# DJjjjhao/FIRA-ICSE

Hardware: NVIDIA H100
Metric: train_commits_per_sec (higher is better)
Workload: dtype bf16

## Files before the change

### fira_icse_b200/csrc/head.cu

```cuda
#include "common.cuh"
#include "fira_b200.h"

namespace {

constexpr int D = 256;
constexpr int TMAX = 32;

__device__ __forceinline__ long src_row(const int* __restrict__ ranges, int b, int S, int s) {
  if (!ranges) return (long)b * S + s;
  const int* r = ranges + 4 * b;
  if (s < r[1]) return r[0] + s;
  s -= r[1];
  return s < r[3] ? (long)(r[2] + s) : -1;
}

template <typename T>
__global__ void __launch_bounds__(256) copy_scores_fwd_kernel(const T* __restrict__ src, const T* __restrict__ tgt,
                                                              const float* __restrict__ w_res,
                                                              const float* __restrict__ b_res_p,
                                                              const unsigned char* __restrict__ src_mask,
                                                              const unsigned char* __restrict__ row_mask,
                                                              const int* __restrict__ ranges,
                                                              float* __restrict__ sc, int B, int Tn, int S) {
  pdl_wait(); pdl_trigger();
// ... 130 lines not shown
struct MaxSum { float m, s; };
__device__ __forceinline__ MaxSum ms_merge(MaxSum a, MaxSum b) {
  const float m = fmaxf(a.m, b.m);
  MaxSum r;
  r.m = m;
  r.s = (a.s == 0.f ? 0.f : a.s * expf(a.m - m)) + (b.s == 0.f ? 0.f : b.s * expf(b.m - m));
  return r;
}
__device__ __forceinline__ MaxSum ms_warp(MaxSum v) {
#pragma unroll
  for (int o = 16; o > 0; o >>= 1) {
    MaxSum u;
    u.m = __shfl_xor_sync(0xffffffffu, v.m, o);
    u.s = __shfl_xor_sync(0xffffffffu, v.s, o);
    v = ms_merge(v, u);
  }
  return v;
}
struct ArgMax { float v; int i; };
__device__ __forceinline__ ArgMax am_better(ArgMax a, ArgMax b) {
  return (b.v > a.v || (b.v == a.v && b.i < a.i)) ? b : a;
}

template <typename T>
__global__ void __launch_bounds__(256) head_fwd_kernel(const T* __restrict__ logits, long ldl,
                                                       const float* __restrict__ sc, const float* __restrict__ gate_logit,
                                                       const unsigned char* __restrict__ mem_mask,
                                                       const int* __restrict__ label, float* __restrict__ stats,
                                                       float* __restrict__ nll, int* __restrict__ argmax_out, int Tn,
                                                       int V, int S) {
  pdl_wait(); pdl_trigger();
  __shared__ MaxSum sh_ms[8];
  __shared__ ArgMax sh_am[8];
  __shared__ float bc[8];
  const long row = blockIdx.x;
  const int b = (int)(row / Tn);
  const int lane = threadIdx.x & 31, warp = threadIdx.x >> 5;
  const T* lrow = logits + row * ldl;
  const float* srow = sc + row * S;
  const unsigned char* mrow = mem_mask + (long)b * S;

  const int lab_row = label[row];
  const bool need_vocab = argmax_out != nullptr || (lab_row != 0 && lab_row < V);
  MaxSum v{-INFINITY, 0.f};
  if (need_vocab) {
    const int V8 = V >> 3;
    for (int g = threadIdx.x; g < V8; g += blockDim.x) {
      float x[8];
      Act<T>::load8(lrow + (long)g * 8, x);
      float m8 = x[0];
#pragma unroll
      for (int i = 1; i < 8; ++i) m8 = fmaxf(m8, x[i]);
      if (m8 > v.m) { v.s *= expf(v.m - m8); v.m = m8; }
#pragma unroll
      for (int i = 0; i < 8; ++i) v.s += expf(x[i] - v.m);
    }
    for (int j = V8 * 8 + threadIdx.x; j < V; j += blockDim.x) { MaxSum u{Act<T>::ld(lrow + j), 1.f}; v = ms_merge(v, u); }
  } else if (threadIdx.x == 0) v = MaxSum{0.f, 1.f};
  v = ms_warp(v);
  if (lane == 0) sh_ms[warp] = v;
  __syncthreads();
  if (warp == 0) { MaxSum u = lane < 8 ? sh_ms[lane] : MaxSum{-INFINITY, 0.f}; u = ms_warp(u); if (lane == 0) { bc[0] = u.m; bc[1] = u.s; } }
  __syncthreads();
  MaxSum c{-INFINITY, 0.f};
  for (int j = threadIdx.x; j < S; j += blockDim.x) { MaxSum u{mrow[j] ? srow[j] : kMaskFill, 1.f}; c = ms_merge(c, u); }
  c = ms_warp(c);
  if (lane == 0) sh_ms[warp] = c;
  __syncthreads();
  if (warp == 0) { MaxSum u = lane < 8 ? sh_ms[lane] : MaxSum{-INFINITY, 0.f}; u = ms_warp(u); if (lane == 0) { bc[2] = u.m; bc[3] = u.s; } }
  __syncthreads();
  const float vmax = bc[0], vsum = bc[1], cmax = bc[2], csum = bc[3];
  const float gl0 = gate_logit[row * 2], gl1 = gate_logit[row * 2 + 1];
  const float gm = fmaxf(gl0, gl1);
  const float e0 = expf(gl0 - gm), e1 = expf(gl1 - gm);
  const float g0 = e0 / (e0 + e1), g1 = e1 / (e0 + e1);

  if (threadIdx.x == 0) {
    const int lab = label[row];
    float p = 1.f;
    if (lab != 0) {
      if (lab < V) p = g0 * (expf(Act<T>::ld(lrow + lab) - vmax) / vsum);
      else {
        const int s = lab - V;
        p = s < S ? g1 * (expf((mrow[s] ? srow[s] : kMaskFill) - cmax) / csum) : 0.f;
      }
    }
    float* st = stats + row * 8;
    st[0] = vmax; st[1] = vsum; st[2] = cmax; st[3] = csum; st[4] = g0; st[5] = g1; st[6] = p; st[7] = 0.f;
    nll[row] = lab != 0 ? -logf(fminf(fmaxf(p, 1e-10f), 1.f)) : 0.f;
  }
  if (argmax_out) {
    ArgMax best{-INFINITY, 0x7fffffff};
    const float iv = 1.f / vsum, ic = 1.f / csum;
    for (int j = threadIdx.x; j < V + S; j += blockDim.x) {
      float p;
      if (j < V) p = g0 * (expf(Act<T>::ld(lrow + j) - vmax) * iv);
      else { const int s = j - V; p = g1 * (expf((mrow[s] ? srow[s] : kMaskFill) - cmax) * ic); }
      ArgMax cand{logf(fminf(fmaxf(p, 1e-10f), 1.f)), j};
      best = am_better(best, cand);
    }
#pragma unroll
    for (int o = 16; o > 0; o >>= 1) {
      ArgMax u{__shfl_xor_sync(0xffffffffu, best.v, o), __shfl_xor_sync(0xffffffffu, best.i, o)};
      best = am_better(best, u);
    }
    if (lane == 0) sh_am[warp] = best;
    __syncthreads();
    if (threadIdx.x == 0) {
      ArgMax r = sh_am[0];
      for (int q = 1; q < 8; ++q) r = am_better(r, sh_am[q]);
      argmax_out[row] = r.i;
    }
  }
}

template <typename T>
__global__ void __launch_bounds__(256) head_bwd_kernel(const T* __restrict__ logits, long ldl,
                                                       const float* __restrict__ sc,
                                                       const unsigned char* __restrict__ mem_mask,
                                                       const int* __restrict__ label, const float* __restrict__ stats,
                                                       const float* __restrict__ upstream, T* __restrict__ d_logits,
                                                       float* __restrict__ d_sc, float* __restrict__ d_gate_logit,
                                                       unsigned char* __restrict__ row_active, int Tn, int V, int S) {
  pdl_wait(); pdl_trigger();
  const long row = blockIdx.x;
  const int b = (int)(row / Tn);
  const float* st = stats + row * 8;
  const float vmax = st[0], vsum = st[1], cmax = st[2], csum = st[3], g0 = st[4], g1 = st[5], p = st[6];
  const int lab = label[row];
  const float up = *upstream;
  const bool live = lab != 0 && p >= 1e-10f && p <= 1.f;
  const bool vocab = live && lab < V;
  const bool copy = live && lab >= V;
  T* drow = d_logits + row * ldl;
  const T* lrow = logits + row * ldl;
  const int V8 = V >> 3;
  if (vocab) {
    const float iv = 1.f / vsum;
    for (int g = threadIdx.x; g < V8; g += blockDim.x) {
      float x[8];
      Act<T>::load8(lrow + (long)g * 8, x);
#pragma unroll
      for (int i = 0; i < 8; ++i) x[i] = up * (expf(x[i] - vmax) * iv - (g * 8 + i == lab ? 1.f : 0.f));
      Act<T>::store8(drow + (long)g * 8, x);
    }
    for (int j = V8 * 8 + threadIdx.x; j < V; j += blockDim.x) {
      float pv = expf(Act<T>::ld(lrow + j) - vmax) * iv;
      Act<T>::st(drow + j, up * (pv - (j == lab ? 1.f : 0.f)));
    }
  } else {
    const float z[8] = {0.f, 0.f, 0.f, 0.f, 0.f, 0.f, 0.f, 0.f};
    for (int g = threadIdx.x; g < V8; g += blockDim.x) Act<T>::store8(drow + (long)g * 8, z);
    for (int j = V8 * 8 + threadIdx.x; j < V; j += blockDim.x) Act<T>::st(drow + j, 0.f);
  }
  const float* srow = sc + row * S;
  const unsigned char* mrow = mem_mask + (long)b * S;
  float* dsrow = d_sc + row * S;
  if (copy) {
    const float ic = 1.f / csum;
    for (int j = threadIdx.x; j < S; j += blockDim.x) {
      float pc = expf((mrow[j] ? srow[j] : kMaskFill) - cmax) * ic;
      dsrow[j] = mrow[j] ? up * (pc - (j == lab - V ? 1.f : 0.f)) : 0.f;
    }
  } else {
    for (int j = threadIdx.x; j < S; j += blockDim.x) dsrow[j] = 0.f;
  }
  if (threadIdx.x == 0) {
    float d0 = 0.f, d1 = 0.f;
    if (vocab) { d0 = up * (g0 - 1.f); d1 = up * g1; }
    if (copy) { d0 = up * g0; d1 = up * (g1 - 1.f); }
    d_gate_logit[row * 2] = d0; d_gate_logit[row * 2 + 1] = d1;
    row_active[row] = copy ? 1 : 0;
  }
}
// ... 632 lines not shown
int fira_copy_scores_bwd(const void* src_proj, const void* tgt_proj, const float* w_res, const float* d_scores,
                         const unsigned char* row_active, void* d_src_proj, float* d_tgt_proj, float* d_w_res,
                         float* d_b_res, int B, int T_len, int S, int dim, int dtype, void* stream) {
  return copy_scores_bwd_impl(src_proj, tgt_proj, w_res, d_scores, row_active, nullptr, d_src_proj, d_tgt_proj, d_w_res,
                              d_b_res, B, T_len, S, dim, dtype, stream);
}

int fira_copy_scores_packed_fwd(const void* src_proj, const void* tgt_proj, const float* w_res, const float* b_res,
                                const int* ranges, const unsigned char* src_mask, const unsigned char* row_mask,
                                float* scores, int B, int T_len, int S, int dim, int dtype, void* stream) {
  FIRA_CHECK_ARG(ranges, FIRA_ERR_ARG, "copy_scores_packed_fwd: null ranges");
  return copy_scores_fwd_impl(src_proj, tgt_proj, w_res, b_res, src_mask, row_mask, ranges, scores, B, T_len, S, dim,
                              dtype, stream);
}

int fira_copy_scores_packed_bwd(const void* src_proj, const void* tgt_proj, const float* w_res, const float* d_scores,
                                const unsigned char* row_active, const int* ranges, void* d_src_proj, float* d_tgt_proj,
                                float* d_w_res, float* d_b_res, int B, int T_len, int S, int dim, int dtype, void* stream) {
  FIRA_CHECK_ARG(ranges, FIRA_ERR_ARG, "copy_scores_packed_bwd: null ranges");
  return copy_scores_bwd_impl(src_proj, tgt_proj, w_res, d_scores, row_active, ranges, d_src_proj, d_tgt_proj, d_w_res,
                              d_b_res, B, T_len, S, dim, dtype, stream);
}

int fira_pointer_mix_nll_fwd(const void* logits, long ld_logits, const float* copy_scores, const float* gate_logits,
                             const unsigned char* mem_mask, const int* label, float* stats, float* nll,
                             int* argmax_out, long rows, int T_len, int V, int S, int dtype, void* stream) {
  FIRA_CHECK_ARG(rows >= 0 && T_len > 0 && V > 0 && S > 0, FIRA_ERR_SHAPE, "pointer_mix_nll_fwd: shape");
  FIRA_CHECK_ARG(fira_aligned16(logits) && ld_logits % 8 == 0, FIRA_ERR_ALIGN,
                 "pointer_mix_nll_fwd: logits must be 16-byte aligned with a leading dimension that is a multiple of 8");
  if (rows == 0) return FIRA_OK;
  DISPATCH_T(dtype, launch_k(head_fwd_kernel<T>, dim3((unsigned)rows), dim3(256), 0, (cudaStream_t)stream, 
      (const T*)logits, ld_logits, copy_scores, gate_logits, mem_mask, label, stats, nll, argmax_out, T_len, V, S);)
  FIRA_CHECK_LAUNCH("fira_pointer_mix_nll_fwd");
  return FIRA_OK;
}

int fira_pointer_mix_nll_bwd(const void* logits, long ld_logits, const float* copy_scores,
                             const unsigned char* mem_mask, const int* label, const float* stats,
                             const float* upstream, void* d_logits, float* d_copy_scores, float* d_gate_logits,
                             unsigned char* row_active, long rows, int T_len, int V, int S, int dtype, void* stream) {
  FIRA_CHECK_ARG(rows >= 0 && T_len > 0 && V > 0 && S > 0, FIRA_ERR_SHAPE, "pointer_mix_nll_bwd: shape");
  FIRA_CHECK_ARG(fira_aligned16(logits) && fira_aligned16(d_logits) && ld_logits % 8 == 0, FIRA_ERR_ALIGN,
                 "pointer_mix_nll_bwd: logits / d_logits must be 16-byte aligned with a leading dimension that is a multiple of 8");
  if (rows == 0) return FIRA_OK;
  DISPATCH_T(dtype, launch_k(head_bwd_kernel<T>, dim3((unsigned)rows), dim3(256), 0, (cudaStream_t)stream, 
      (const T*)logits, ld_logits, copy_scores, mem_mask, label, stats, upstream, (T*)d_logits, d_copy_scores,
      d_gate_logits, row_active, T_len, V, S);)
  FIRA_CHECK_LAUNCH("fira_pointer_mix_nll_bwd");
  return FIRA_OK;
}

static int sample_impl(const void* logits, long ld_logits, const float* copy_scores, const float* gate_logits,
                       const unsigned char* mem_mask, const int* copy_src, const uint64_t* seed, const int* first_index,
                       const float* uniforms, float temperature, int top_k, float top_p, int eos_id, int pad_id,
                       int* next_tok, int* seq, int* raw, float* token_logprob, unsigned char* tok_mask, long ld_out,
                       int pos, unsigned char* finished, int* length, float* logprob, int B, int N, int V, int S,
                       const int* prefix, int ld_prefix, const int* prefix_len, int no_repeat, int min_len, int dtype,
                       void* stream) {
  FIRA_CHECK_ARG(!prefix || (prefix_len && ld_prefix > pos), FIRA_ERR_ARG,
                 "pointer_mix_sample_prefix: null prefix_len or ld_prefix %d <= pos %d", ld_prefix, pos);
  FIRA_CHECK_ARG(no_repeat >= 0 && min_len >= 0, FIRA_ERR_ARG,
                 "pointer_mix_sample_rules: no_repeat_ngram %d / min_length %d < 0", no_repeat, min_len);
  FIRA_CHECK_ARG((!no_repeat && !min_len) || ld_out <= TMAX, FIRA_ERR_SHAPE,
                 "pointer_mix_sample_rules: ld_out %ld > %d", ld_out, TMAX);
  FIRA_CHECK_ARG(B >= 0 && N > 0 && V > 0 && S > 0 && V + S <= 0x7FFF, FIRA_ERR_SHAPE,
                 "pointer_mix_sample: shape (B %d, N %d, V %d, S %d; V + S must be <= 32767)", B, N, V, S);
  FIRA_CHECK_ARG(pos >= 0 && ld_out >= pos + 2, FIRA_ERR_SHAPE, "pointer_mix_sample: pos %d, ld_out %ld", pos, ld_out);
  FIRA_CHECK_ARG(temperature > 0.f && temperature <= 3.4e38f, FIRA_ERR_ARG, "pointer_mix_sample: temperature %g",
                 (double)temperature);
  FIRA_CHECK_ARG(top_k >= 0, FIRA_ERR_ARG, "pointer_mix_sample: top_k %d < 0", top_k);
  FIRA_CHECK_ARG(top_p > 0.f && top_p <= 1.f, FIRA_ERR_ARG, "pointer_mix_sample: top_p %g not in (0, 1]", (double)top_p);
  FIRA_CHECK_ARG(uniforms || (seed && first_index), FIRA_ERR_ARG, "pointer_mix_sample: seed / first_index missing");
// ... 215 lines not shown
```

### fira_icse_b200/data.py

```python
import json
import os
import random

import numpy as np
import torch
from torch.utils.data import Dataset

from ._lib import host_call

num_train, num_valid, num_test = 75000, 8000, 7661
lemmatization = {"added": "add", "fixed": "fix", "removed": "remove",
                 "adding": "add", "fixing": "fix", "removing": "remove"}
RAW_FILES = ["difftoken", "diffatt", "diffmark", "msg", "variable", "change", "ast",
             "edge_change_code", "edge_change_ast", "edge_ast_code", "edge_ast"]


def _lower(tok, upper):
    return tok if tok in upper else tok.lower()


def _to_ids(tokens, vocab, upper):
    out = []
    for t in tokens:
        t = _lower(t, upper)
# ... 301 lines not shown

    def __len__(self):
        n = len(self.indices)
        return n // self.B if self.drop_last else -(-n // self.B)

    def _choose_dims(self, need):
        need = tuple(int(x) for x in need)
        if need in self.shapes or self.max_shapes is None or len(self.shapes) < self.max_shapes:
            self.shapes[need] = self.shapes.get(need, 0) + 1
            return need
        fits = [s for s in self.shapes if all(a >= b for a, b in zip(s, need))]
        if self.packed and not fits:
            self.shapes[need] = 1
            return need
        best = min(fits, key=sum) if fits else self.lens
        self.shapes[best] = self.shapes.get(best, 0) + 1
        return best

    def gather(self, index, slot=None):
        slot = self.slots[0] if slot is None else slot
        index = np.ascontiguousarray(index, dtype=np.int64)
        if self.packed:
            from . import packed as P
            need = self.tables.dims(index)
            want = tuple(P._round_up(need[i], self.row_buckets[i]) for i in range(4))
            return P.gather_packed(self.tables, index, self.V, slot, pad_dims=self._choose_dims(want))
        b = len(index)
        n0, n1, n2 = self.lens
        t = self.tab
        dims = np.zeros(3, np.int32)
        host_call("fira_host_batch_dims", t["sou"].ctypes.data, t["sub_token"].ctypes.data,
                  t["ast_change"].ctypes.data, index.ctypes.data, b, n0, n1, n2, *self.multiples, dims.ctypes.data)
        dims = np.asarray(self._choose_dims(dims), np.int32)
        nnz = np.zeros(1, np.int32)
        host_call("fira_host_gather_batch", t["sou"].ctypes.data, t["tar"].ctypes.data, t["mark"].ctypes.data,
                  t["ast_change"].ctypes.data, t["tar_label"].ctypes.data, t["sub_token"].ctypes.data,
                  self.deg.ctypes.data, self.col.ctypes.data, self.val.ctypes.data, self.edge_ptr.ctypes.data,
                  index.ctypes.data, b, n0, n1, n2, self.msg_len, self.V, dims.ctypes.data,
                  slot.sou.data_ptr(), slot.tar.data_ptr(), slot.mark.data_ptr(), slot.ast_change.data_ptr(),
                  slot.tar_label.data_ptr(), slot.sub_token.data_ptr(), slot.rowptr.data_ptr(), slot.col.data_ptr(),
                  slot.val.data_ptr(), self.edge_cap, nnz.ctypes.data)
        c0, c1, c2 = (int(x) for x in dims)
        e = int(nnz[0])
        slot.batch = [slot.sou[:b * c0].view(b, c0), slot.tar[:b * self.msg_len].view(b, self.msg_len), None,
                      slot.mark[:b * c0].view(b, c0), slot.ast_change[:b * c2].view(b, c2),
                      (slot.rowptr[:b * (c0 + c1 + c2) + 1], slot.col[:e], slot.val[:e]),
                      slot.tar_label[:b * self.msg_len].view(b, self.msg_len), slot.sub_token[:b * c1].view(b, c1)]
        return slot.batch
# ... 71 lines not shown
```

### fira_icse_b200/engine.py

```python
import os

import torch
import torch.distributed as dist

from . import optim as _optim
from .graph import PackedEdges
from .optim import FlatAdam
from .packed import PackedBatch
from .parallel import FlatGradBucket

ID_KEYS = ("sou", "tar", "mark", "ast_change", "tar_label", "sub_token")


class _Captured:

    def __init__(self, shapes, B, n_nodes, cap, dev):
        self.ids = {k: torch.zeros((B, n), dtype=torch.int64, device=dev) for k, n in zip(ID_KEYS, shapes)}
        self.rowptr = torch.zeros(B * n_nodes + 1, dtype=torch.int32, device=dev)
        self.col = torch.zeros(cap, dtype=torch.int32, device=dev)
        self.val = torch.zeros(cap, dtype=torch.float32, device=dev)
        self.B, self.n_nodes, self.cap = B, n_nodes, cap
        self.graph = None
        self.grads = None


class _CapturedPacked:

    def __init__(self, pb, cap, dev):
        def z(t, n=None):
            return torch.zeros(t.shape if n is None else (n,), dtype=t.dtype, device=dev)
        t = {k: z(getattr(pb, k)) for k in PackedBatch.FIELDS if k not in ("col", "val")}
        t["col"], t["val"] = z(pb.col, cap), z(pb.val, cap)
        self.pb = PackedBatch(pb.B, pb.Rc, pb.Rs, pb.Ra, pb.S, pb.T, cap, pb.chunks, **t)
        self.B, self.cap = pb.B, cap
        self.graph = None
        self.grads = None
        self.packed = True

    def copy_from(self, pb):
        for k in PackedBatch.FIELDS:
            src, dst = getattr(pb, k), getattr(self.pb, k)
            if k in ("col", "val"):
                dst[:src.numel()].copy_(src, non_blocking=True)
            else:
                dst.copy_(src, non_blocking=True)


class _OptimizerPair:

    def __init__(self, pair):
        self.pair = pair

    def step(self):
        for o in self.pair:
            o.step()

# ... 326 lines not shown
```

### fira_icse_b200/ops.py

```python
import ctypes
import os

import torch

from . import _lib
from . import optim as _optim
from ._lib import FIRA_BF16, FIRA_F32, call

D = 256

if hasattr(torch.autograd.graph, "set_warn_on_accumulate_grad_stream_mismatch"):
    torch.autograd.graph.set_warn_on_accumulate_grad_stream_mismatch(False)


def _stream():
    return torch.cuda.current_stream().cuda_stream


def _ptr(t, off=0):
    if t is None:
        return None
    return t.data_ptr() + off * t.element_size()


# ... 689 lines not shown

class HeadFn(torch.autograd.Function):

    @staticmethod
    def forward(ctx, want_argmax, bf16, pf, memory, dec, mem_mask, label, Wout, bout, Ws, Wt, Wres, bres, Wp, bp,
                pk=None):
        _require_cuda(memory, dec, Wout)
        B, T = dec.shape[0], dec.shape[1]
        S = pk.S if pk is not None else memory.shape[1]
        V = Wout.shape[0]
        Mt, Ms = B * T, memory.shape[0] * memory.shape[1]
        pr = Prec(bf16)
        if pf is not None and pf.event is not None:
            torch.cuda.current_stream().wait_event(pf.event)
            pf.fork.join()
            pr.wcache.update(pf.wcache)
        dev = dec.device
        f32 = dict(dtype=torch.float32, device=dev)
        st = _stream()
        memory2 = memory.contiguous().to(pr.tdt).view(Ms, D)
        dec2 = dec.contiguous().to(pr.tdt).view(Mt, D)
        dec32 = dec2 if not pr.bf16 else dec2.float()
        ldl = _ld_logits(V)
        logits = pr.empty((Mt, ldl), dev)
        pr.linear(dec2, Wout, bout, out=logits, ld_out=ldl)
        row_mask = None if want_argmax else (label >= V).to(torch.uint8)
        src, tgt, sc = copy_scores_fwd(pr, memory2, dec2, Ws, Wt, Wres, bres, B, T, S, src_mask=mem_mask,
                                       row_mask=row_mask, ranges=pk.ranges if pk is not None else None)
        gl = linear(dec32, Wp, bp)
        stats = torch.empty((Mt, 8), **f32)
        nll = torch.empty((Mt,), **f32)
        amax = torch.empty((Mt,), dtype=torch.int32, device=dev) if want_argmax else None
        call("fira_pointer_mix_nll_fwd", _ptr(logits), ldl, _ptr(sc), _ptr(gl), _ptr(mem_mask), _ptr(label),
             _ptr(stats), _ptr(nll), _ptr(amax), Mt, T, V, S, pr.code, st)
        ctx.misc = (pr, memory2, dec2, dec32, mem_mask, label, logits, ldl, src, tgt, sc, stats, B, T, S, V,
                    memory.dtype, dec.dtype, pk, memory.shape)
        ctx.save_for_backward(Wout, Ws, Wt, Wres, Wp, bout, bres, bp)
        loss_sum = colsum(nll, 1, Mt, 1).view(())
        ids = amax.view(B, T) if want_argmax else None
        nll2 = nll.view(B, T)
        ctx.mark_non_differentiable(*([nll2, ids] if ids is not None else [nll2]))
        return loss_sum, nll2, ids

    @staticmethod
    def backward(ctx, g_loss, g_nll, g_ids):
        (pr, memory2, dec2, dec32, mem_mask, label, logits, ldl, src, tgt, sc, stats, B, T, S, V,
         mem_dt, dec_dt, pk, mem_shape) = ctx.misc
        Wout, Ws, Wt, Wres, Wp, bout, bres, bp = ctx.saved_tensors
        Mt, Ms = B * T, memory2.shape[0]
        dev = dec2.device
        f32 = dict(dtype=torch.float32, device=dev)
        st = _stream()
        up = g_loss.contiguous().float()
        dlogits = pr.empty((Mt, ldl), dev)
        dsc = torch.empty((B, T, S), **f32)
        dgl = torch.empty((Mt, 2), **f32)
        active = torch.empty((Mt,), dtype=torch.uint8, device=dev)
        call("fira_pointer_mix_nll_bwd", _ptr(logits), ldl, _ptr(sc), _ptr(mem_mask), _ptr(label), _ptr(stats),
             _ptr(up), _ptr(dlogits), _ptr(dsc), _ptr(dgl), _ptr(active), Mt, T, V, S, pr.code, st)
        d_src = pr.empty((Ms, D), dev)
        d_tgt = torch.zeros((Mt, D), **f32)
        d_wres = _gdest(Wres, (1, D), zero=True)
        d_bres = _gdest(bres, (1,), zero=True)
        if pk is not None:
            call("fira_zero_pad_rows", _ptr(d_src), D, D, _ptr(pk.off), B, pk.Rc, pk.Rs, pr.code, st)
            call("fira_copy_scores_packed_bwd", _ptr(src), _ptr(tgt), _ptr(Wres), _ptr(dsc), _ptr(active), _ptr(pk.ranges),
                 _ptr(d_src), _ptr(d_tgt), _ptr(d_wres), _ptr(d_bres), B, T, S, D, pr.code, st)
        else:
            call("fira_copy_scores_bwd", _ptr(src), _ptr(tgt), _ptr(Wres), _ptr(dsc), _ptr(active), _ptr(d_src),
                 _ptr(d_tgt), _ptr(d_wres), _ptr(d_bres), B, T, S, D, pr.code, st)
        fork = Fork(dev)
        with fork(d_src, memory2):
            d_Ws = pr.linear_dw(d_src, D, memory2, D, Ms, D, D, out=_gdest(Ws, (D, D)))
        with fork(dlogits, dec2):
            d_bout = _gdest(bout, (V,), zero=True)
            d_Wout = pr.linear_dw(dlogits, ldl, dec2, D, Mt, V, D, out=_gdest(Wout, (V, D)), dbias=d_bout)
        with fork(dgl, dec32, d_tgt):
            d_bp = colsum(dgl, 2, Mt, 2, out=_gdest(bp, (2,), zero=True))
            d_Wp = linear_dw(dgl, 2, dec32, D, Mt, 2, D, out=_gdest(Wp, (2, D)))
            d_Wt = linear_dw(d_tgt, D, dec32, D, Mt, D, D, out=_gdest(Wt, (D, D)))
        d_mem = pr.linear_dx(d_src, D, Ws, Ms)
        if pr.bf16:
            d_dec = torch.empty((Mt, D), **f32)
            gemm_tc(dlogits, ldl, 1, pr.w(Wout), D, 0, d_dec, D, Mt, D, V,
                    splits=_tc_splits(_ceil(Mt, 128), _ceil(V, 64)))
        else:
            d_dec = linear_dx(dlogits, ldl, Wout, Mt)
        linear_dx(dgl, 2, Wp, Mt, out=d_dec, accumulate=True)
        linear_dx(d_tgt, D, Wt, Mt, out=d_dec, accumulate=True)
        fork.join()
        return (None, None, None, d_mem.view(mem_shape).to(mem_dt), d_dec.view(B, T, D).to(dec_dt), None, None, d_Wout,
                d_bout, d_Ws, d_Wt, d_wres, d_bres, d_Wp, d_bp, None)


class LinearFn(torch.autograd.Function):

    @staticmethod
    def forward(ctx, x, W, b):
        _require_cuda(x, W)
        N, K = W.shape
        x2 = x.contiguous().float().view(-1, K)
        M = x2.shape[0]
        ld = (N + 3) // 4 * 4
        out = torch.empty((M, ld), dtype=torch.float32, device=x.device)
        linear(x2, W, b, out=out, ld_out=ld)
        ctx.save_for_backward(x2, W)
        ctx.has_bias = b is not None
        ctx.shape = x.shape
        return out[:, :N].view(*x.shape[:-1], N)

# ... 46 lines not shown
```

### fira_icse_b200/packed.py

```python
import numpy as np
import torch

from ._lib import host_call

SEGMENT_BUCKETS = (1024, 512, 512, 64)


class PackedBatch:

    FIELDS = ("code", "mark", "pos", "sub", "ast", "off", "ranges", "mem_mask", "tar", "label", "tar_mask",
              "rowptr", "col", "val")

    def __init__(self, B, Rc, Rs, Ra, S, T, nnz, chunks=4, **tensors):
        self.B, self.Rc, self.Rs, self.Ra, self.S, self.T, self.nnz = B, Rc, Rs, Ra, S, T, nnz
        self.chunks = int(chunks)
        for k in self.FIELDS:
            setattr(self, k, tensors[k])

    @property
    def shape_key(self):
        return (self.B, self.Rc, self.Rs, self.Ra, self.S, self.chunks)

    @property
    def rows(self):
        return self.Rc + self.Rs + self.Ra

    @property
    def mem_rows(self):
        return self.Rc + self.Rs

    def to(self, device, non_blocking=True):
        t = {k: getattr(self, k).to(device, non_blocking=non_blocking) for k in self.FIELDS}
        return PackedBatch(self.B, self.Rc, self.Rs, self.Ra, self.S, self.T, self.nnz, self.chunks, **t)

    def h2d_bytes(self):
        return sum(getattr(self, k).numel() * getattr(self, k).element_size() for k in self.FIELDS)


def _round_up(x, m):
    return max(m, -(-int(x) // m) * m)


class PackedTables:

    ID_KEYS = ("sou", "tar", "mark", "ast_change", "tar_label", "sub_token")

    def __init__(self, dataset):
        d = dataset.d
        self.tab = {k: np.ascontiguousarray(d[k], dtype=np.int32) for k in self.ID_KEYS}
        self.deg = np.ascontiguousarray(d["deg"], dtype=np.uint8)
        self.col = np.ascontiguousarray(d["col"], dtype=np.int16)
        self.val = np.ascontiguousarray(d["val"], dtype=np.float64)
        self.edge_ptr = np.ascontiguousarray(d["edge_ptr"], dtype=np.int64)
        self.lens = (dataset.diff_len, dataset.sub_token_len, dataset.ast_change_len)
        self.msg_len = dataset.msg_len
        self.n = len(self.tab["sou"])

    def dims(self, index):
        index = np.ascontiguousarray(index, dtype=np.int64)
        t = self.tab
        out = np.zeros(6, np.int32)
        host_call("fira_host_packed_dims", t["sou"].ctypes.data, t["sub_token"].ctypes.data, t["ast_change"].ctypes.data,
                  self.deg.ctypes.data, index.ctypes.data, len(index), *self.lens, out.ctypes.data)
        return tuple(int(x) for x in out)


class PackedSlot:

    def __init__(self, B, lens, msg_len, edge_cap, pin):
        n0, n1, n2 = lens

        def buf(n, dt):
            t = torch.empty(n, dtype=dt)
            return t.pin_memory() if pin else t
        i32, u8 = torch.int32, torch.uint8
        self.cap = (_round_up(B * n0, SEGMENT_BUCKETS[0]), _round_up(B * n1, SEGMENT_BUCKETS[1]),
                    _round_up(B * n2, SEGMENT_BUCKETS[2]), _round_up(n0 + n1, SEGMENT_BUCKETS[3]))
        Rc, Rs, Ra, S = self.cap
        self.code, self.mark, self.pos = buf(Rc, i32), buf(Rc, i32), buf(Rc, i32)
        self.sub, self.ast = buf(Rs, i32), buf(Ra, i32)
        self.off, self.ranges = buf(3 * (B + 1), i32), buf(4 * B, i32)
        self.mem_mask = buf(B * S, u8)
        self.tar, self.label, self.tar_mask = buf(B * msg_len, i32), buf(B * msg_len, i32), buf(B * msg_len, u8)
        self.rowptr = buf(Rc + Rs + Ra + 1, i32)
        self.col, self.val = buf(edge_cap, i32), buf(edge_cap, torch.float32)
        self.edge_cap = edge_cap
        self.event = None
        self.batch = None


def gather_packed(tables, index, vocab_size, slot, pad_dims=None, buckets=SEGMENT_BUCKETS):
    index = np.ascontiguousarray(index, dtype=np.int64)
    b = len(index)
    need = tables.dims(index)
    if pad_dims is None:
        pad_dims = tuple(_round_up(need[i], buckets[i]) for i in range(4))
    Rc, Rs, Ra, S = (int(x) for x in pad_dims)
    if Rc > slot.cap[0] or Rs > slot.cap[1] or Ra > slot.cap[2] or S > slot.cap[3]:
        raise ValueError(f"packed batch {pad_dims} exceeds the staging capacity {slot.cap}")
    t = tables.tab
    pd = np.asarray((Rc, Rs, Ra, S), np.int32)
    nnz = np.zeros(1, np.int32)
    host_call("fira_host_gather_packed", t["sou"].ctypes.data, t["tar"].ctypes.data, t["mark"].ctypes.data,
              t["ast_change"].ctypes.data, t["tar_label"].ctypes.data, t["sub_token"].ctypes.data,
              tables.deg.ctypes.data, tables.col.ctypes.data, tables.val.ctypes.data, tables.edge_ptr.ctypes.data,
              index.ctypes.data, b, *tables.lens, tables.msg_len, int(vocab_size), pd.ctypes.data,
              slot.code.data_ptr(), slot.mark.data_ptr(), slot.pos.data_ptr(), slot.sub.data_ptr(), slot.ast.data_ptr(),
              slot.off.data_ptr(), slot.ranges.data_ptr(), slot.mem_mask.data_ptr(), slot.tar.data_ptr(),
              slot.label.data_ptr(), slot.tar_mask.data_ptr(), slot.rowptr.data_ptr(), slot.col.data_ptr(),
              slot.val.data_ptr(), slot.edge_cap, nnz.ctypes.data)
    e, T = int(nnz[0]), tables.msg_len
    slot.batch = PackedBatch(
        b, Rc, Rs, Ra, S, T, e, max(3, need[5]),
        code=slot.code[:Rc], mark=slot.mark[:Rc], pos=slot.pos[:Rc], sub=slot.sub[:Rs], ast=slot.ast[:Ra],
        off=slot.off[:3 * (b + 1)].view(3, b + 1), ranges=slot.ranges[:4 * b].view(b, 4),
        mem_mask=slot.mem_mask[:b * S].view(b, S), tar=slot.tar[:b * T].view(b, T), label=slot.label[:b * T].view(b, T),
        tar_mask=slot.tar_mask[:b * T].view(b, T), rowptr=slot.rowptr[:Rc + Rs + Ra + 1], col=slot.col[:e],
        val=slot.val[:e])
    return slot.batch


def pack_from_dataset(dataset, index, vocab_size, pin=False, pad_dims=None, buckets=SEGMENT_BUCKETS):
    tables = dataset if isinstance(dataset, PackedTables) else PackedTables(dataset)
    per_commit = int(np.diff(tables.edge_ptr).max()) if len(tables.edge_ptr) > 1 else 0
    slot = PackedSlot(len(index), tables.lens, tables.msg_len, max(1, per_commit * len(index)), pin)
    return gather_packed(tables, index, vocab_size, slot, pad_dims=pad_dims, buckets=buckets)
```

### include/fira_b200.h

```cpp
#ifndef FIRA_B200_H_
#define FIRA_B200_H_

#include <stdint.h>

#ifdef __cplusplus
extern "C" {
#endif

#define FIRA_F32 0
#define FIRA_BF16 1
#define FIRA_EDGE_F32 0
#define FIRA_EDGE_BF16 1
#define FIRA_EDGE_F64 2

int fira_version(void);
const char* fira_last_error_string(void);
int fira_built_arch(void);
int fira_num_sms(void);
int fira_set_pdl(int on);
int fira_get_pdl(void);

int fira_gemm_f32(const float* A, long lda, int a_kcontig, const float* B, long ldb, int b_kcontig, float* C,
                  long ldc, int M, int N, int K, const float* bias, const float* rs, const float* rc, int relu,
                  int accumulate, int splits, void* stream);
// ... 99 lines not shown
                     uint32_t stream_id, void* stream);

int fira_copy_scores_fwd(const void* src_proj, const void* tgt_proj, const float* w_res, const float* b_res,
                         const unsigned char* src_mask, const unsigned char* row_mask, float* scores,
                         int B, int T_len, int S, int dim, int dtype, void* stream);
int fira_copy_scores_bwd(const void* src_proj, const void* tgt_proj, const float* w_res, const float* d_scores,
                         const unsigned char* row_active, void* d_src_proj, float* d_tgt_proj, float* d_w_res,
                         float* d_b_res, int B, int T_len, int S, int dim, int dtype, void* stream);

int fira_copy_scores_packed_fwd(const void* src_proj, const void* tgt_proj, const float* w_res, const float* b_res,
                                const int* ranges, const unsigned char* src_mask, const unsigned char* row_mask,
                                float* scores, int B, int T_len, int S, int dim, int dtype, void* stream);
int fira_copy_scores_packed_bwd(const void* src_proj, const void* tgt_proj, const float* w_res, const float* d_scores,
                                const unsigned char* row_active, const int* ranges, void* d_src_proj, float* d_tgt_proj,
                                float* d_w_res, float* d_b_res, int B, int T_len, int S, int dim, int dtype, void* stream);

int fira_pointer_mix_nll_fwd(const void* logits, long ld_logits, const float* copy_scores, const float* gate_logits,
                             const unsigned char* mem_mask, const int* label, float* stats, float* nll,
                             int* argmax_out, long rows, int T_len, int V, int S, int dtype, void* stream);
int fira_pointer_mix_nll_bwd(const void* logits, long ld_logits, const float* copy_scores,
                             const unsigned char* mem_mask, const int* label, const float* stats,
                             const float* upstream, void* d_logits, float* d_copy_scores, float* d_gate_logits,
                             unsigned char* row_active, long rows, int T_len, int V, int S, int dtype, void* stream);

int fira_pointer_mix_sample(const void* logits, long ld_logits, const float* copy_scores, const float* gate_logits,
                            const unsigned char* mem_mask, const int* copy_src, const uint64_t* seed,
                            const int* first_index, const float* uniforms, float temperature, int top_k, float top_p,
                            int eos_id, int pad_id, int* next_tok, int* seq, int* raw, float* token_logprob,
                            unsigned char* tok_mask, long ld_out, int pos, unsigned char* finished, int* length,
                            float* logprob, int B, int N, int V, int S, int dtype, void* stream);

int fira_pointer_mix_beam_step(const void* logits, long ld_logits, const float* copy_scores, const float* gate_logits,
                               const unsigned char* mem_mask, const int* copy_src, float length_penalty, int eos_id,
                               int pad_id, uint64_t* workspace, int* seq, int* raw, float* token_logprob, int* length,
                               float* logprob, float* score, unsigned char* status, long* parent, int* next_tok,
                               int T_len, int pos, int B, int K, int V, int S, int dtype, void* stream);

int fira_pointer_mix_diverse_beam_step(const void* logits, long ld_logits, const float* copy_scores,
                                       const float* gate_logits, const unsigned char* mem_mask, const int* copy_src,
                                       float length_penalty, int eos_id, int pad_id, uint64_t* workspace, int* seq,
                                       int* raw, float* token_logprob, int* length, float* logprob, float* score,
                                       unsigned char* status, long* parent, int* next_tok, int T_len, int pos, int B,
                                       int K, int V, int S, int groups, float diversity, int* chosen,
                                       float* lp_workspace, int dtype, void* stream);

int fira_pointer_mix_sample_prefix(const void* logits, long ld_logits, const float* copy_scores,
// ... 81 lines not shown
```

Measured before the change: 20060.

## Compute vocabulary logits only for rows whose label is a vocabulary token

Adds a compaction kernel that lists the decoder rows whose label falls in the vocabulary, gathers those decoder states, and runs the output projection GEMM, head forward/backward, and weight/input gradient GEMMs only on that compacted set, sized by a host-side bucketed count. The aim is to avoid vocab-sized logits work for padding and copy-labelled rows, which contribute nothing to the loss gradient. In exchange it adds a single-block scan kernel, two gather launches, a per-batch count computed on the host, and another shape dimension that may trigger recompilation or graph recapture.

```diff
diff --git a/fira_icse_b200/csrc/head.cu b/fira_icse_b200/csrc/head.cu
--- a/fira_icse_b200/csrc/head.cu
+++ b/fira_icse_b200/csrc/head.cu
@@ -176,13 +176,55 @@
   return (b.v > a.v || (b.v == a.v && b.i < a.i)) ? b : a;
 }
 
+constexpr int kRowsThreads = 1024;
+__global__ void __launch_bounds__(kRowsThreads) vocab_rows_kernel(const int* __restrict__ label, long rows, int V,
+                                                                  int* __restrict__ vslot, int* __restrict__ vrows,
+                                                                  int cap) {
+  pdl_wait(); pdl_trigger();
+  __shared__ int warp_sum_s[kRowsThreads / 32];
+  const int lane = threadIdx.x & 31, warp = threadIdx.x >> 5;
+  const long per = (rows + kRowsThreads - 1) / kRowsThreads;
+  const long r0 = min(rows, (long)threadIdx.x * per), r1 = min(rows, r0 + per);
+  int n = 0;
+  for (long r = r0; r < r1; ++r) n += (label[r] != 0 && label[r] < V);
+  int incl = n;
+#pragma unroll
+  for (int o = 1; o < 32; o <<= 1) { const int u = __shfl_up_sync(0xffffffffu, incl, o); if (lane >= o) incl += u; }
+  if (lane == 31) warp_sum_s[warp] = incl;
+  for (int s = threadIdx.x; s < cap; s += kRowsThreads) vrows[s] = -1;
+  __syncthreads();
+  int slot = incl - n;
+  for (int w = 0; w < warp; ++w) slot += warp_sum_s[w];
+  for (long r = r0; r < r1; ++r) {
+    const bool v = label[r] != 0 && label[r] < V && slot < cap;
+    vslot[r] = v ? slot : -1;
+    if (v) vrows[slot++] = (int)r;
+  }
+}
+
+template <typename T>
+__global__ void __launch_bounds__(256) gather_rows_kernel(const T* __restrict__ src, long ld_src,
+                                                          const int* __restrict__ idx, T* __restrict__ dst, long ld_dst,
+                                                          long n, int width) {
+  pdl_wait(); pdl_trigger();
+  const int lane = threadIdx.x & 31;
+  for (long i = (long)blockIdx.x * 8 + (threadIdx.x >> 5); i < n; i += (long)gridDim.x * 8) {
+    const int r = idx[i];
+    for (int c = lane * 8; c < width; c += 256) {
+      float x[8] = {0.f, 0.f, 0.f, 0.f, 0.f, 0.f, 0.f, 0.f};
+      if (r >= 0) Act<T>::load8(src + (long)r * ld_src + c, x);
+      Act<T>::store8(dst + i * ld_dst + c, x);
+    }
+  }
+}
+
 template <typename T>
 __global__ void __launch_bounds__(256) head_fwd_kernel(const T* __restrict__ logits, long ldl,
                                                        const float* __restrict__ sc, const float* __restrict__ gate_logit,
                                                        const unsigned char* __restrict__ mem_mask,
-                                                       const int* __restrict__ label, float* __restrict__ stats,
-                                                       float* __restrict__ nll, int* __restrict__ argmax_out, int Tn,
-                                                       int V, int S) {
+                                                       const int* __restrict__ label, const int* __restrict__ vslot,
+                                                       float* __restrict__ stats, float* __restrict__ nll,
+                                                       int* __restrict__ argmax_out, int Tn, int V, int S) {
   pdl_wait(); pdl_trigger();
   __shared__ MaxSum sh_ms[8];
   __shared__ ArgMax sh_am[8];
@@ -190,12 +232,13 @@
   const long row = blockIdx.x;
   const int b = (int)(row / Tn);
   const int lane = threadIdx.x & 31, warp = threadIdx.x >> 5;
-  const T* lrow = logits + row * ldl;
+  const long lslot = vslot ? (long)vslot[row] : row;
+  const T* lrow = logits + lslot * ldl;
   const float* srow = sc + row * S;
   const unsigned char* mrow = mem_mask + (long)b * S;
 
   const int lab_row = label[row];
-  const bool need_vocab = argmax_out != nullptr || (lab_row != 0 && lab_row < V);
+  const bool need_vocab = argmax_out != nullptr || (lab_row != 0 && lab_row < V && lslot >= 0);
   MaxSum v{-INFINITY, 0.f};
   if (need_vocab) {
     const int V8 = V >> 3;
@@ -232,8 +275,9 @@
   if (threadIdx.x == 0) {
     const int lab = label[row];
     float p = 1.f;
+    const bool no_slot = lab != 0 && lab < V && lslot < 0;
     if (lab != 0) {
-      if (lab < V) p = g0 * (expf(Act<T>::ld(lrow + lab) - vmax) / vsum);
+      if (lab < V) p = no_slot ? NAN : g0 * (expf(Act<T>::ld(lrow + lab) - vmax) / vsum);
       else {
         const int s = lab - V;
         p = s < S ? g1 * (expf((mrow[s] ? srow[s] : kMaskFill) - cmax) / csum) : 0.f;
@@ -241,7 +285,7 @@
     }
     float* st = stats + row * 8;
     st[0] = vmax; st[1] = vsum; st[2] = cmax; st[3] = csum; st[4] = g0; st[5] = g1; st[6] = p; st[7] = 0.f;
-    nll[row] = lab != 0 ? -logf(fminf(fmaxf(p, 1e-10f), 1.f)) : 0.f;
+    nll[row] = no_slot ? NAN : (lab != 0 ? -logf(fminf(fmaxf(p, 1e-10f), 1.f)) : 0.f);
   }
   if (argmax_out) {
     ArgMax best{-INFINITY, 0x7fffffff};
@@ -272,7 +316,9 @@
 __global__ void __launch_bounds__(256) head_bwd_kernel(const T* __restrict__ logits, long ldl,
                                                        const float* __restrict__ sc,
                                                        const unsigned char* __restrict__ mem_mask,
-                                                       const int* __restrict__ label, const float* __restrict__ stats,
+                                                       const int* __restrict__ label, const int* __restrict__ vslot,
+                                                       const int* __restrict__ vrows, int cap,
+                                                       const float* __restrict__ stats,
                                                        const float* __restrict__ upstream, T* __restrict__ d_logits,
                                                        float* __restrict__ d_sc, float* __restrict__ d_gate_logit,
                                                        unsigned char* __restrict__ row_active, int Tn, int V, int S) {
@@ -284,11 +330,18 @@
   const int lab = label[row];
   const float up = *upstream;
   const bool live = lab != 0 && p >= 1e-10f && p <= 1.f;
-  const bool vocab = live && lab < V;
+  const long lslot = vslot ? (long)vslot[row] : row;
+  const bool vocab = live && lab < V && lslot >= 0;
   const bool copy = live && lab >= V;
-  T* drow = d_logits + row * ldl;
-  const T* lrow = logits + row * ldl;
+  T* drow = d_logits + lslot * ldl;
+  const T* lrow = logits + lslot * ldl;
   const int V8 = V >> 3;
+  const float z[8] = {0.f, 0.f, 0.f, 0.f, 0.f, 0.f, 0.f, 0.f};
+  if (vslot && row < cap && vrows[row] < 0) {
+    T* prow = d_logits + row * ldl;
+    for (int g = threadIdx.x; g < V8; g += blockDim.x) Act<T>::store8(prow + (long)g * 8, z);
+    for (int j = V8 * 8 + threadIdx.x; j < V; j += blockDim.x) Act<T>::st(prow + j, 0.f);
+  }
   if (vocab) {
     const float iv = 1.f / vsum;
     for (int g = threadIdx.x; g < V8; g += blockDim.x) {
@@ -302,8 +355,7 @@
       float pv = expf(Act<T>::ld(lrow + j) - vmax) * iv;
       Act<T>::st(drow + j, up * (pv - (j == lab ? 1.f : 0.f)));
     }
-  } else {
-    const float z[8] = {0.f, 0.f, 0.f, 0.f, 0.f, 0.f, 0.f, 0.f};
+  } else if (lslot >= 0) {
     for (int g = threadIdx.x; g < V8; g += blockDim.x) Act<T>::store8(drow + (long)g * 8, z);
     for (int j = V8 * 8 + threadIdx.x; j < V; j += blockDim.x) Act<T>::st(drow + j, 0.f);
   }
@@ -982,16 +1034,64 @@
                               d_b_res, B, T_len, S, dim, dtype, stream);
 }
 
+int fira_vocab_rows(const int* label, long rows, int V, int* vslot, int* vrows, int cap, void* stream) {
+  FIRA_CHECK_ARG(label && vslot && vrows && rows >= 0 && V > 0 && cap >= 0, FIRA_ERR_ARG, "vocab_rows: arguments");
+  launch_k(vocab_rows_kernel, dim3(1), dim3(kRowsThreads), 0, (cudaStream_t)stream, label, rows, V, vslot, vrows, cap);
+  FIRA_CHECK_LAUNCH("fira_vocab_rows");
+  return FIRA_OK;
+}
+
+int fira_gather_rows(const void* src, long ld_src, const int* idx, void* dst, long ld_dst, long n, int width, int dtype,
+                     void* stream) {
+  FIRA_CHECK_ARG(idx && n >= 0 && width > 0 && width % 8 == 0 && ld_src >= width && ld_dst >= width, FIRA_ERR_ARG,
+                 "gather_rows: arguments");
+  FIRA_CHECK_ARG(fira_aligned16(src) && fira_aligned16(dst) && ld_src % 8 == 0 && ld_dst % 8 == 0, FIRA_ERR_ALIGN,
+                 "gather_rows: 16-B alignment");
+  if (n == 0) return FIRA_OK;
+  const long g = (n + 7) / 8, gmax = (long)fira_num_sms() * 16;
+  DISPATCH_T(dtype, launch_k(gather_rows_kernel<T>, dim3((unsigned)(g < gmax ? g : gmax)), dim3(256), 0,
+      (cudaStream_t)stream, (const T*)src, ld_src, idx, (T*)dst, ld_dst, n, width);)
+  FIRA_CHECK_LAUNCH("fira_gather_rows");
+  return FIRA_OK;
+}
+
+int fira_pointer_mix_nll_fwd_rows(const void* logits, long ld_logits, const float* copy_scores, const float* gate_logits,
+                                  const unsigned char* mem_mask, const int* label, const int* vslot, float* stats,
+                                  float* nll, int* argmax_out, long rows, int T_len, int V, int S, int dtype,
+                                  void* stream) {
+  FIRA_CHECK_ARG(rows >= 0 && T_len > 0 && V > 0 && S > 0, FIRA_ERR_SHAPE, "pointer_mix_nll_fwd: shape");
+  FIRA_CHECK_ARG(fira_aligned16(logits) && ld_logits % 8 == 0, FIRA_ERR_ALIGN,
+                 "pointer_mix_nll_fwd: logits must be 16-byte aligned with a leading dimension that is a multiple of 8");
+  FIRA_CHECK_ARG(!(vslot && argmax_out), FIRA_ERR_ARG, "pointer_mix_nll_fwd: the argmax needs the logits of every row");
+  if (rows == 0) return FIRA_OK;
+  DISPATCH_T(dtype, launch_k(head_fwd_kernel<T>, dim3((unsigned)rows), dim3(256), 0, (cudaStream_t)stream,
+      (const T*)logits, ld_logits, copy_scores, gate_logits, mem_mask, label, vslot, stats, nll, argmax_out, T_len, V,
+      S);)
+  FIRA_CHECK_LAUNCH("fira_pointer_mix_nll_fwd");
+  return FIRA_OK;
+}
+
 int fira_pointer_mix_nll_fwd(const void* logits, long ld_logits, const float* copy_scores, const float* gate_logits,
                              const unsigned char* mem_mask, const int* label, float* stats, float* nll,
                              int* argmax_out, long rows, int T_len, int V, int S, int dtype, void* stream) {
-  FIRA_CHECK_ARG(rows >= 0 && T_len > 0 && V > 0 && S > 0, FIRA_ERR_SHAPE, "pointer_mix_nll_fwd: shape");
-  FIRA_CHECK_ARG(fira_aligned16(logits) && ld_logits % 8 == 0, FIRA_ERR_ALIGN,
-                 "pointer_mix_nll_fwd: logits must be 16-byte aligned with a leading dimension that is a multiple of 8");
+  return fira_pointer_mix_nll_fwd_rows(logits, ld_logits, copy_scores, gate_logits, mem_mask, label, nullptr, stats, nll,
+                                       argmax_out, rows, T_len, V, S, dtype, stream);
+}
+
+int fira_pointer_mix_nll_bwd_rows(const void* logits, long ld_logits, const float* copy_scores,
+                                  const unsigned char* mem_mask, const int* label, const int* vslot, const int* vrows,
+                                  int cap, const float* stats, const float* upstream, void* d_logits,
+                                  float* d_copy_scores, float* d_gate_logits, unsigned char* row_active, long rows,
+                                  int T_len, int V, int S, int dtype, void* stream) {
+  FIRA_CHECK_ARG(rows >= 0 && T_len > 0 && V > 0 && S > 0, FIRA_ERR_SHAPE, "pointer_mix_nll_bwd: shape");
+  FIRA_CHECK_ARG(fira_aligned16(logits) && fira_aligned16(d_logits) && ld_logits % 8 == 0, FIRA_ERR_ALIGN,
+                 "pointer_mix_nll_bwd: logits / d_logits must be 16-byte aligned with a leading dimension that is a multiple of 8");
+  FIRA_CHECK_ARG(!vslot || (vrows && cap >= 0 && cap <= rows), FIRA_ERR_ARG, "pointer_mix_nll_bwd: vrows / cap");
   if (rows == 0) return FIRA_OK;
-  DISPATCH_T(dtype, launch_k(head_fwd_kernel<T>, dim3((unsigned)rows), dim3(256), 0, (cudaStream_t)stream, 
-      (const T*)logits, ld_logits, copy_scores, gate_logits, mem_mask, label, stats, nll, argmax_out, T_len, V, S);)
-  FIRA_CHECK_LAUNCH("fira_pointer_mix_nll_fwd");
+  DISPATCH_T(dtype, launch_k(head_bwd_kernel<T>, dim3((unsigned)rows), dim3(256), 0, (cudaStream_t)stream,
+      (const T*)logits, ld_logits, copy_scores, mem_mask, label, vslot, vrows, cap, stats, upstream, (T*)d_logits,
+      d_copy_scores, d_gate_logits, row_active, T_len, V, S);)
+  FIRA_CHECK_LAUNCH("fira_pointer_mix_nll_bwd");
   return FIRA_OK;
 }
 
@@ -999,15 +1099,9 @@
                              const unsigned char* mem_mask, const int* label, const float* stats,
                              const float* upstream, void* d_logits, float* d_copy_scores, float* d_gate_logits,
                              unsigned char* row_active, long rows, int T_len, int V, int S, int dtype, void* stream) {
-  FIRA_CHECK_ARG(rows >= 0 && T_len > 0 && V > 0 && S > 0, FIRA_ERR_SHAPE, "pointer_mix_nll_bwd: shape");
-  FIRA_CHECK_ARG(fira_aligned16(logits) && fira_aligned16(d_logits) && ld_logits % 8 == 0, FIRA_ERR_ALIGN,
-                 "pointer_mix_nll_bwd: logits / d_logits must be 16-byte aligned with a leading dimension that is a multiple of 8");
-  if (rows == 0) return FIRA_OK;
-  DISPATCH_T(dtype, launch_k(head_bwd_kernel<T>, dim3((unsigned)rows), dim3(256), 0, (cudaStream_t)stream, 
-      (const T*)logits, ld_logits, copy_scores, mem_mask, label, stats, upstream, (T*)d_logits, d_copy_scores,
-      d_gate_logits, row_active, T_len, V, S);)
-  FIRA_CHECK_LAUNCH("fira_pointer_mix_nll_bwd");
-  return FIRA_OK;
+  return fira_pointer_mix_nll_bwd_rows(logits, ld_logits, copy_scores, mem_mask, label, nullptr, nullptr, 0, stats,
+                                       upstream, d_logits, d_copy_scores, d_gate_logits, row_active, rows, T_len, V, S,
+                                       dtype, stream);
 }
 
 static int sample_impl(const void* logits, long ld_logits, const float* copy_scores, const float* gate_logits,
diff --git a/fira_icse_b200/data.py b/fira_icse_b200/data.py
--- a/fira_icse_b200/data.py
+++ b/fira_icse_b200/data.py
@@ -347,8 +347,7 @@
         index = np.ascontiguousarray(index, dtype=np.int64)
         if self.packed:
             from . import packed as P
-            need = self.tables.dims(index)
-            want = tuple(P._round_up(need[i], self.row_buckets[i]) for i in range(4))
+            want = P.packed_needs(self.tables, index, self.V, self.row_buckets)
             return P.gather_packed(self.tables, index, self.V, slot, pad_dims=self._choose_dims(want))
         b = len(index)
         n0, n1, n2 = self.lens
diff --git a/fira_icse_b200/engine.py b/fira_icse_b200/engine.py
--- a/fira_icse_b200/engine.py
+++ b/fira_icse_b200/engine.py
@@ -31,7 +31,7 @@
             return torch.zeros(t.shape if n is None else (n,), dtype=t.dtype, device=dev)
         t = {k: z(getattr(pb, k)) for k in PackedBatch.FIELDS if k not in ("col", "val")}
         t["col"], t["val"] = z(pb.col, cap), z(pb.val, cap)
-        self.pb = PackedBatch(pb.B, pb.Rc, pb.Rs, pb.Ra, pb.S, pb.T, cap, pb.chunks, **t)
+        self.pb = PackedBatch(pb.B, pb.Rc, pb.Rs, pb.Ra, pb.S, pb.T, cap, pb.chunks, pb.Rv, **t)
         self.B, self.cap = pb.B, cap
         self.graph = None
         self.grads = None
diff --git a/fira_icse_b200/ops.py b/fira_icse_b200/ops.py
--- a/fira_icse_b200/ops.py
+++ b/fira_icse_b200/ops.py
@@ -735,8 +735,17 @@
         dec2 = dec.contiguous().to(pr.tdt).view(Mt, D)
         dec32 = dec2 if not pr.bf16 else dec2.float()
         ldl = _ld_logits(V)
-        logits = pr.empty((Mt, ldl), dev)
-        pr.linear(dec2, Wout, bout, out=logits, ld_out=ldl)
+        if want_argmax:
+            cap, vslot, vrows, dec_v = Mt, None, None, dec2
+        else:
+            cap = Mt if pk is None else pk.Rv
+            vslot = torch.empty((Mt,), dtype=torch.int32, device=dev)
+            vrows = torch.empty((cap,), dtype=torch.int32, device=dev)
+            call("fira_vocab_rows", _ptr(label), Mt, V, _ptr(vslot), _ptr(vrows), cap, st)
+            dec_v = pr.empty((cap, D), dev)
+            call("fira_gather_rows", _ptr(dec2), D, _ptr(vrows), _ptr(dec_v), D, cap, D, pr.code, st)
+        logits = pr.empty((cap, ldl), dev)
+        pr.linear(dec_v, Wout, bout, out=logits, ld_out=ldl)
         row_mask = None if want_argmax else (label >= V).to(torch.uint8)
         src, tgt, sc = copy_scores_fwd(pr, memory2, dec2, Ws, Wt, Wres, bres, B, T, S, src_mask=mem_mask,
                                        row_mask=row_mask, ranges=pk.ranges if pk is not None else None)
@@ -744,10 +753,10 @@
         stats = torch.empty((Mt, 8), **f32)
         nll = torch.empty((Mt,), **f32)
         amax = torch.empty((Mt,), dtype=torch.int32, device=dev) if want_argmax else None
-        call("fira_pointer_mix_nll_fwd", _ptr(logits), ldl, _ptr(sc), _ptr(gl), _ptr(mem_mask), _ptr(label),
-             _ptr(stats), _ptr(nll), _ptr(amax), Mt, T, V, S, pr.code, st)
+        call("fira_pointer_mix_nll_fwd_rows", _ptr(logits), ldl, _ptr(sc), _ptr(gl), _ptr(mem_mask), _ptr(label),
+             _ptr(vslot), _ptr(stats), _ptr(nll), _ptr(amax), Mt, T, V, S, pr.code, st)
         ctx.misc = (pr, memory2, dec2, dec32, mem_mask, label, logits, ldl, src, tgt, sc, stats, B, T, S, V,
-                    memory.dtype, dec.dtype, pk, memory.shape)
+                    memory.dtype, dec.dtype, pk, memory.shape, cap, vslot, vrows, dec_v)
         ctx.save_for_backward(Wout, Ws, Wt, Wres, Wp, bout, bres, bp)
         loss_sum = colsum(nll, 1, Mt, 1).view(())
         ids = amax.view(B, T) if want_argmax else None
@@ -758,19 +767,20 @@
     @staticmethod
     def backward(ctx, g_loss, g_nll, g_ids):
         (pr, memory2, dec2, dec32, mem_mask, label, logits, ldl, src, tgt, sc, stats, B, T, S, V,
-         mem_dt, dec_dt, pk, mem_shape) = ctx.misc
+         mem_dt, dec_dt, pk, mem_shape, cap, vslot, vrows, dec_v) = ctx.misc
         Wout, Ws, Wt, Wres, Wp, bout, bres, bp = ctx.saved_tensors
         Mt, Ms = B * T, memory2.shape[0]
         dev = dec2.device
         f32 = dict(dtype=torch.float32, device=dev)
         st = _stream()
         up = g_loss.contiguous().float()
-        dlogits = pr.empty((Mt, ldl), dev)
+        dlogits = pr.empty((cap, ldl), dev)
         dsc = torch.empty((B, T, S), **f32)
         dgl = torch.empty((Mt, 2), **f32)
         active = torch.empty((Mt,), dtype=torch.uint8, device=dev)
-        call("fira_pointer_mix_nll_bwd", _ptr(logits), ldl, _ptr(sc), _ptr(mem_mask), _ptr(label), _ptr(stats),
-             _ptr(up), _ptr(dlogits), _ptr(dsc), _ptr(dgl), _ptr(active), Mt, T, V, S, pr.code, st)
+        call("fira_pointer_mix_nll_bwd_rows", _ptr(logits), ldl, _ptr(sc), _ptr(mem_mask), _ptr(label), _ptr(vslot),
+             _ptr(vrows), cap, _ptr(stats), _ptr(up), _ptr(dlogits), _ptr(dsc), _ptr(dgl), _ptr(active), Mt, T, V, S,
+             pr.code, st)
         d_src = pr.empty((Ms, D), dev)
         d_tgt = torch.zeros((Mt, D), **f32)
         d_wres = _gdest(Wres, (1, D), zero=True)
@@ -785,20 +795,23 @@
         fork = Fork(dev)
         with fork(d_src, memory2):
             d_Ws = pr.linear_dw(d_src, D, memory2, D, Ms, D, D, out=_gdest(Ws, (D, D)))
-        with fork(dlogits, dec2):
+        with fork(dlogits, dec_v):
             d_bout = _gdest(bout, (V,), zero=True)
-            d_Wout = pr.linear_dw(dlogits, ldl, dec2, D, Mt, V, D, out=_gdest(Wout, (V, D)), dbias=d_bout)
+            d_Wout = pr.linear_dw(dlogits, ldl, dec_v, D, cap, V, D, out=_gdest(Wout, (V, D)), dbias=d_bout)
         with fork(dgl, dec32, d_tgt):
             d_bp = colsum(dgl, 2, Mt, 2, out=_gdest(bp, (2,), zero=True))
             d_Wp = linear_dw(dgl, 2, dec32, D, Mt, 2, D, out=_gdest(Wp, (2, D)))
             d_Wt = linear_dw(d_tgt, D, dec32, D, Mt, D, D, out=_gdest(Wt, (D, D)))
         d_mem = pr.linear_dx(d_src, D, Ws, Ms)
         if pr.bf16:
-            d_dec = torch.empty((Mt, D), **f32)
-            gemm_tc(dlogits, ldl, 1, pr.w(Wout), D, 0, d_dec, D, Mt, D, V,
-                    splits=_tc_splits(_ceil(Mt, 128), _ceil(V, 64)))
+            d_dec = torch.empty((cap, D), **f32)
+            gemm_tc(dlogits, ldl, 1, pr.w(Wout), D, 0, d_dec, D, cap, D, V,
+                    splits=_tc_splits(_ceil(cap, 128), _ceil(V, 64)))
         else:
-            d_dec = linear_dx(dlogits, ldl, Wout, Mt)
+            d_dec = linear_dx(dlogits, ldl, Wout, cap)
+        if vslot is not None:
+            d_dec_v, d_dec = d_dec, torch.empty((Mt, D), **f32)
+            call("fira_gather_rows", _ptr(d_dec_v), D, _ptr(vslot), _ptr(d_dec), D, Mt, D, FIRA_F32, st)
         linear_dx(dgl, 2, Wp, Mt, out=d_dec, accumulate=True)
         linear_dx(d_tgt, D, Wt, Mt, out=d_dec, accumulate=True)
         fork.join()
diff --git a/fira_icse_b200/packed.py b/fira_icse_b200/packed.py
--- a/fira_icse_b200/packed.py
+++ b/fira_icse_b200/packed.py
@@ -4,6 +4,7 @@
 from ._lib import host_call
 
 SEGMENT_BUCKETS = (1024, 512, 512, 64)
+VOCAB_ROW_BUCKET = 128
 
 
 class PackedBatch:
@@ -11,15 +12,16 @@
     FIELDS = ("code", "mark", "pos", "sub", "ast", "off", "ranges", "mem_mask", "tar", "label", "tar_mask",
               "rowptr", "col", "val")
 
-    def __init__(self, B, Rc, Rs, Ra, S, T, nnz, chunks=4, **tensors):
+    def __init__(self, B, Rc, Rs, Ra, S, T, nnz, chunks=4, Rv=None, **tensors):
         self.B, self.Rc, self.Rs, self.Ra, self.S, self.T, self.nnz = B, Rc, Rs, Ra, S, T, nnz
         self.chunks = int(chunks)
+        self.Rv = B * T if Rv is None else int(Rv)
         for k in self.FIELDS:
             setattr(self, k, tensors[k])
 
     @property
     def shape_key(self):
-        return (self.B, self.Rc, self.Rs, self.Ra, self.S, self.chunks)
+        return (self.B, self.Rc, self.Rs, self.Ra, self.S, self.chunks, self.Rv)
 
     @property
     def rows(self):
@@ -31,7 +33,7 @@
 
     def to(self, device, non_blocking=True):
         t = {k: getattr(self, k).to(device, non_blocking=non_blocking) for k in self.FIELDS}
-        return PackedBatch(self.B, self.Rc, self.Rs, self.Ra, self.S, self.T, self.nnz, self.chunks, **t)
+        return PackedBatch(self.B, self.Rc, self.Rs, self.Ra, self.S, self.T, self.nnz, self.chunks, self.Rv, **t)
 
     def h2d_bytes(self):
         return sum(getattr(self, k).numel() * getattr(self, k).element_size() for k in self.FIELDS)
@@ -64,6 +66,10 @@
                   self.deg.ctypes.data, index.ctypes.data, len(index), *self.lens, out.ctypes.data)
         return tuple(int(x) for x in out)
 
+    def vocab_rows(self, index, vocab_size):
+        lab = self.tab["tar_label"][np.asarray(index, dtype=np.int64), 1:]
+        return int(np.count_nonzero((lab > 0) & (lab < vocab_size)))
+
 
 class PackedSlot:
 
@@ -94,10 +100,14 @@
     b = len(index)
     need = tables.dims(index)
     if pad_dims is None:
-        pad_dims = tuple(_round_up(need[i], buckets[i]) for i in range(4))
-    Rc, Rs, Ra, S = (int(x) for x in pad_dims)
+        pad_dims = packed_needs(tables, index, vocab_size, buckets)
+    elif len(pad_dims) == 4:
+        pad_dims = tuple(pad_dims) + packed_needs(tables, index, vocab_size, buckets)[4:]
+    Rc, Rs, Ra, S, Rv = (int(x) for x in pad_dims)
     if Rc > slot.cap[0] or Rs > slot.cap[1] or Ra > slot.cap[2] or S > slot.cap[3]:
         raise ValueError(f"packed batch {pad_dims} exceeds the staging capacity {slot.cap}")
+    if Rv < tables.vocab_rows(index, vocab_size):
+        raise ValueError(f"packed batch: Rv = {Rv} is below its vocabulary-label rows")
     t = tables.tab
     pd = np.asarray((Rc, Rs, Ra, S), np.int32)
     nnz = np.zeros(1, np.int32)
@@ -111,7 +121,7 @@
               slot.val.data_ptr(), slot.edge_cap, nnz.ctypes.data)
     e, T = int(nnz[0]), tables.msg_len
     slot.batch = PackedBatch(
-        b, Rc, Rs, Ra, S, T, e, max(3, need[5]),
+        b, Rc, Rs, Ra, S, T, e, max(3, need[5]), min(Rv, b * T),
         code=slot.code[:Rc], mark=slot.mark[:Rc], pos=slot.pos[:Rc], sub=slot.sub[:Rs], ast=slot.ast[:Ra],
         off=slot.off[:3 * (b + 1)].view(3, b + 1), ranges=slot.ranges[:4 * b].view(b, 4),
         mem_mask=slot.mem_mask[:b * S].view(b, S), tar=slot.tar[:b * T].view(b, T), label=slot.label[:b * T].view(b, T),
@@ -120,6 +130,12 @@
     return slot.batch
 
 
+def packed_needs(tables, index, vocab_size, buckets=SEGMENT_BUCKETS):
+    need = tables.dims(index)
+    return tuple(_round_up(need[i], buckets[i]) for i in range(4)) + \
+        (_round_up(tables.vocab_rows(index, vocab_size), VOCAB_ROW_BUCKET),)
+
+
 def pack_from_dataset(dataset, index, vocab_size, pin=False, pad_dims=None, buckets=SEGMENT_BUCKETS):
     tables = dataset if isinstance(dataset, PackedTables) else PackedTables(dataset)
     per_commit = int(np.diff(tables.edge_ptr).max()) if len(tables.edge_ptr) > 1 else 0
diff --git a/include/fira_b200.h b/include/fira_b200.h
--- a/include/fira_b200.h
+++ b/include/fira_b200.h
@@ -145,6 +145,19 @@
                              const unsigned char* mem_mask, const int* label, const float* stats,
                              const float* upstream, void* d_logits, float* d_copy_scores, float* d_gate_logits,
                              unsigned char* row_active, long rows, int T_len, int V, int S, int dtype, void* stream);
+
+int fira_vocab_rows(const int* label, long rows, int V, int* vslot, int* vrows, int cap, void* stream);
+int fira_gather_rows(const void* src, long ld_src, const int* idx, void* dst, long ld_dst, long n, int width, int dtype,
+                     void* stream);
+int fira_pointer_mix_nll_fwd_rows(const void* logits, long ld_logits, const float* copy_scores, const float* gate_logits,
+                                  const unsigned char* mem_mask, const int* label, const int* vslot, float* stats,
+                                  float* nll, int* argmax_out, long rows, int T_len, int V, int S, int dtype,
+                                  void* stream);
+int fira_pointer_mix_nll_bwd_rows(const void* logits, long ld_logits, const float* copy_scores,
+                                  const unsigned char* mem_mask, const int* label, const int* vslot, const int* vrows,
+                                  int cap, const float* stats, const float* upstream, void* d_logits,
+                                  float* d_copy_scores, float* d_gate_logits, unsigned char* row_active, long rows,
+                                  int T_len, int V, int S, int dtype, void* stream);
 
 int fira_pointer_mix_sample(const void* logits, long ld_logits, const float* copy_scores, const float* gate_logits,
                             const unsigned char* mem_mask, const int* copy_src, const uint64_t* seed,
```

Result: faster. 21250 (median of 6 runs) (+5.9%).
